# NVlabs/EmerNeRF

Measured on AMD Instinct MI355X. Metric: train rays/sec (8192-ray batch, 128 samples), higher is better.
Workload: dtype f32

## Files before the change

### emernerf_amd/csrc/mlp_fused.hip

```cpp
#include <type_traits>

#include "common.h"
#include "bf16x3.h"

namespace emer {

constexpr int kNThreads = 512;
constexpr int kNeckChunk = 8;

struct WSrc {
    const float *w;
    int64_t sn, sk;
    int32_t n, k;
};

template <int KS> struct Opd { u32x4 h[KS], m[KS], l[KS]; };

template <int KT>
__device__ __forceinline__ void make_opd(const f32x4 (&in)[KT], Opd<(KT + 1) / 2> &o) {
#pragma unroll
    for (int s = 0; s < (KT + 1) / 2; ++s) {
#pragma unroll
        for (int q = 0; q < 4; ++q) {
            const int t = 2 * s + (q >> 1), e = 2 * (q & 1);
// ... 1414 lines not shown
            } else {
                set_kstep(xo, 0, x[0], x[1]);
#pragma unroll
                for (int p = 0; p < 4; ++p) {
                    a1[p] = *reinterpret_cast<const f32x4 *>(rb + 16 * p + 4 * g);
                    a2[p] = *reinterpret_cast<const f32x4 *>(rb + 64 + 16 * p + 4 * g);
                }
                EMER_RGBW_SB();
                ld_frag6(fb, w1gf, 0, 0); mma_frag6<2>(fa, xo, 0, a1[0], a1[1]);
                set_kstep(xo, 1, x[2], x[3]);
                EMER_RGBW_SB();
                ld_frag6(fa, w0f, 0, 1); mma_frag6<2>(fb, xo, 0, a2[0], a2[1]);
                EMER_RGBW_SB();
                ld_frag6(fb, w1gf, 0, 1); mma_frag6<2>(fa, xo, 0, a1[2], a1[3]);
                EMER_RGBW_SB();
                ld_frag6(fa, w0f, 1, 0); mma_frag6<2>(fb, xo, 0, a2[2], a2[3]);
                EMER_RGBW_SB();
                ld_frag6(fb, w1gf, 1, 0); mma_frag6<2>(fa, xo, 1, a1[0], a1[1]);
                EMER_RGBW_SB();
                ld_frag6(fa, w0f, 1, 1); mma_frag6<2>(fb, xo, 1, a2[0], a2[1]);
                {
                    f32x4 v[2] = {a1[0], a1[1]};
                    relu<2>(v);
                    a1[0] = v[0]; a1[1] = v[1];
                    set_kstep(ho, 0, v[0], v[1]);
                }
                EMER_RGBW_SB();
                ld_frag6(fb, w1gf, 1, 1); mma_frag6<2>(fa, xo, 1, a1[2], a1[3]);
                EMER_RGBW_SB();
                ld_frag6(fa, w1af, 0, 0); mma_frag6<2>(fb, xo, 1, a2[2], a2[3]);
                {
                    f32x4 v[2] = {a1[2], a1[3]};
                    relu<2>(v);
                    a1[2] = v[0]; a1[3] = v[1];
                    set_kstep(ho, 1, v[0], v[1]);
                }
                EMER_RGBW_SB();
                ld_frag6(fb, w1af, 0, 1); mma_frag6<2>(fa, ho, 0, a2[0], a2[1]);
                Bq[2] = block32(to_rows<2>(xo, 0, sel), to_rows<2>(xo, 1, sel));
                EMER_RGBW_SB();
                ld_frag6(fa, w1af, 1, 0); mma_frag6<2>(fb, ho, 0, a2[2], a2[3]);
                Bq[3] = block32(to_rows<2>(xo, 2, sel), to_rows<2>(xo, 3, sel));
                EMER_RGBW_SB();
                ld_frag6(fb, w1af, 1, 1); mma_frag6<2>(fa, ho, 1, a2[0], a2[1]);
                Bq[0] = block32(to_rows<2>(ho, 0, sel), to_rows<2>(ho, 1, sel));
                EMER_RGBW_SB();
                ld_frag6(fa, L.w1a, 0, 0); mma_frag6<2>(fb, ho, 1, a2[2], a2[3]);
                Bq[1] = block32(to_rows<2>(ho, 2, sel), to_rows<2>(ho, 3, sel));
                EMER_RGBW_SB();
            }
            relu<4>(a2);
            Opd<2> d1o, d0o;
            f32x4 dg[4];
            rgb_w_chain(st, L, fa, fb, wfirst, d2, a2,
                        [&](f32x4 (&m1)[4]) {
#pragma unroll
                            for (int p = 0; p < 4; ++p) m1[p] = a1[p];
                        },
                        [](int) {}, d1o, d0o, dg);
#pragma unroll
            for (int p = 0; p < 4; ++p) dgp[p] = dg[p];
            dgeo_prev = dgeo;
            EMER_RGBW_SB();
            rgb_w_products(st, sel, d1o, d0o, Bq, s1c, s0c);
        }
        rgb_w_store_sums(a, L, ray, s1c, s0c);
        rpar ^= 1;
    }
    rgb_w_store_dgeo(dgeo_prev, dgp, L.lo64);
    rgb_w_epilogue(st, a, L, smem);
}

struct DensBwdWArgs {
    const float *ddens, *dens, *enc; int64_t n; int32_t n_levels;
    WSrc w0; const float *b0; const float *w1;
    float *denc;
    float *partials; int64_t stride;
};
constexpr int kDensPartMax = 64 * 16 + 64 + 64 + 4;

template <int KS4>
__global__ __launch_bounds__(kNThreads, 2) void density_bwdw_kernel(const DensBwdWArgs a, int32_t F) {
    __shared__ float part[kNThreads / 64][kDensPartMax];
    const int wave = __builtin_amdgcn_readfirstlane(threadIdx.x >> 6), lane = threadIdx.x & 63, m = lane & 15, g = lane >> 4;
    const int32_t K0 = a.w0.k;
    float aw[4][KS4];
    int64_t koff[KS4];
#pragma unroll
    for (int s = 0; s < KS4; ++s) {
        const int32_t k = 4 * s + g, kc = k < K0 ? k : K0 - 1;
        koff[s] = (int64_t)(kc / F) * a.n * F + kc % F;
#pragma unroll
        for (int p = 0; p < 4; ++p) aw[p][s] = k < K0 ? a.w0.w[(int64_t)(16 * p + m) * a.w0.sn + (int64_t)k * a.w0.sk] : 0.0f;
    }
    f32x4 b0r[4], w1r[4], awt[4];
#pragma unroll
    for (int p = 0; p < 4; ++p)
#pragma unroll
        for (int i = 0; i < 4; ++i) {
            const int32_t nf = 16 * p + 4 * g + i;
            b0r[p][i] = a.b0 ? a.b0[nf] : 0.0f;
            w1r[p][i] = a.w1[nf];
            awt[p][i] = m < K0 ? a.w0.w[(int64_t)nf * a.w0.sn + (int64_t)m * a.w0.sk] : 0.0f;
        }
    float w0acc[4 * KS4], w1acc = 0.0f, b0acc = 0.0f, b1acc = 0.0f;
#pragma unroll
    for (int k = 0; k < 4 * KS4; ++k) w0acc[k] = 0.0f;
    const int64_t n_tiles = (a.n + 15) >> 4, n_chunks = (n_tiles + kNeckChunk - 1) / kNeckChunk;
    for (int64_t c = (int64_t)blockIdx.x * (blockDim.x >> 6) + wave; c < n_chunks; c += (int64_t)gridDim.x * (blockDim.x >> 6)) {
        const int64_t t0 = c * kNeckChunk;
        float x[kNeckChunk][KS4], dd[kNeckChunk], de[kNeckChunk];
#pragma unroll
        for (int j = 0; j < kNeckChunk; ++j) {
            const int64_t row = (t0 + j) * 16 + m, rc = row < a.n ? row : a.n - 1;
#pragma unroll
            for (int s = 0; s < KS4; ++s) x[j][s] = a.enc[koff[s] + rc * F];
            dd[j] = a.ddens[rc];
            de[j] = a.dens[rc];
        }
#pragma unroll
        for (int j = 0; j < kNeckChunk; ++j) {
            if (t0 + j >= n_tiles) break;
            const int64_t row = (t0 + j) * 16 + m;
            const bool ok = row < a.n;
            f32x4 h[4];
#pragma unroll
            for (int p = 0; p < 4; ++p) h[p] = b0r[p];
#pragma unroll
            for (int s = 0; s < KS4; ++s)
#pragma unroll
                for (int p = 0; p < 4; ++p) h[p] = __builtin_amdgcn_mfma_f32_16x16x4f32(aw[p][s], x[j][s], h[p], 0, 0, 0);
            relu<4>(h);
            const float fix = ok ? trunc_exp_bwd(dd[j], de[j]) : 0.0f;
            f32x4 dh[4];
#pragma unroll
            for (int p = 0; p < 4; ++p)
#pragma unroll
                for (int i = 0; i < 4; ++i) dh[p][i] = h[p][i] > 0.0f ? w1r[p][i] * fix : 0.0f;
            f32x4 dx = {0.0f, 0.0f, 0.0f, 0.0f};
#pragma unroll
            for (int p = 0; p < 4; ++p)
#pragma unroll
                for (int i = 0; i < 4; ++i) dx = __builtin_amdgcn_mfma_f32_16x16x4f32(awt[p][i], dh[p][i], dx, 0, 0, 0);
            if (ok)
#pragma unroll
                for (int r = 0; r < 4; ++r) {
                    const int32_t k = 4 * g + r;
                    if (k < K0) a.denc[(int64_t)(k / F) * a.n * F + row * F + k % F] = dx[r];
                }
            w1acc += row16_reduce_scatter(h, fix, m);
            b0acc += row16_reduce_scatter(dh, 1.0f, m);
            if (g == 0) b1acc += fix;
#pragma unroll
            for (int k = 0; k < 4 * KS4; ++k) {
                const float ek = __shfl(x[j][k >> 2], 16 * (k & 3) + m, 64);
                w0acc[k] += row16_reduce_scatter(dh, ek, m);
                __builtin_amdgcn_sched_barrier(0);
            }
        }
    }
    const int nf = 16 * (m >> 2) + 4 * g + (m & 3);
#pragma unroll
    for (int k = 0; k < 4 * KS4; ++k)
        if (k < K0) part[wave][nf * K0 + k] = w0acc[k];
    part[wave][64 * K0 + nf] = b0acc;
    part[wave][64 * K0 + 64 + nf] = w1acc;
    b1acc = row16_sum(b1acc);
    if (lane == 0) part[wave][64 * K0 + 128] = b1acc;
    __syncthreads();
    const int total = 64 * K0 + 129;
    for (int i = threadIdx.x; i < total; i += (int)blockDim.x) {
        float t = 0.0f;
        for (int w = 0; w < (int)(blockDim.x >> 6); ++w) t += part[w][i];
        a.partials[(int64_t)blockIdx.x * a.stride + i] = t;
    }
}

struct RMlpFwdArgs {
    const float *x; int64_t ldx;
    int64_t n; int32_t n_levels, k0, n_out, final_act;
    WSrc w0, w1, w2; const float *b0, *b1, *b2;
    float *h1, *h2;
    float *out; int64_t ldo;
};

template <int KT>
__device__ __forceinline__ void ld_rm_k(const float *rowp, bool ok, int g, int k0, f32x4 (&v)[KT]) {
#pragma unroll
    for (int t = 0; t < KT; ++t)
        v[t] = (ok && 16 * t + 4 * g < k0) ? *reinterpret_cast<const f32x4 *>(rowp + t * 16 + 4 * g) : f32x4{0.0f, 0.0f, 0.0f, 0.0f};
}
template <int KT>
__device__ __forceinline__ void st_rm_k(float *rowp, bool ok, int g, int k0, const f32x4 (&v)[KT]) {
    if (!ok) return;
#pragma unroll
    for (int t = 0; t < KT; ++t)
        if (16 * t + 4 * g < k0) *reinterpret_cast<f32x4 *>(rowp + t * 16 + 4 * g) = v[t];
}
template <int NT>
__device__ __forceinline__ void ld_narrow(const float *rowp, bool ok, int g, int n_valid, f32x4 (&v)[NT]) {
#pragma unroll
    for (int p = 0; p < NT; ++p)
#pragma unroll
        for (int i = 0; i < 4; ++i) v[p][i] = (ok && 16 * p + 4 * g + i < n_valid) ? rowp[16 * p + 4 * g + i] : 0.0f;
}
template <int NT>
__device__ __forceinline__ void st_narrow(float *rowp, bool ok, int g, int n_valid, const f32x4 (&v)[NT]) {
    if (!ok) return;
#pragma unroll
    for (int p = 0; p < NT; ++p)
#pragma unroll
        for (int i = 0; i < 4; ++i)
            if (16 * p + 4 * g + i < n_valid) rowp[16 * p + 4 * g + i] = v[p][i];
}

template <int KT0, int NL, int NTO>
struct RMlpFwdLds {
    static constexpr int KS0 = (KT0 + 1) / 2, NP1 = NL == 3 ? 4 : NTO;
    static constexpr int w0 = 0, w1 = w0 + w3_units(4, KS0), w2 = w1 + w3_units(NP1, 2), fl = w2 + (NL == 3 ? w3_units(NTO, 2) : 0);
    static constexpr int b0 = 0, b1 = b0 + 64, b2 = b1 + 64, n_fl = b2 + 64;
    static constexpr size_t bytes = (size_t)fl * 16 + n_fl * sizeof(float);
};

template <int KT0, int F, int NL, int NTO>
__global__ __launch_bounds__(kNThreads, 4) void rmlp_fwd_kernel(const RMlpFwdArgs a) {
    extern __shared__ __attribute__((aligned(16))) u32x4 smem[];
    using Lds = RMlpFwdLds<KT0, NL, NTO>;
    constexpr int KS0 = Lds::KS0, NP1 = Lds::NP1;
    u32x4 *w0l = smem + Lds::w0, *w1l = smem + Lds::w1, *w2l = smem + Lds::w2;
    float *fl = reinterpret_cast<float *>(smem + Lds::fl), *b0l = fl + Lds::b0, *b1l = fl + Lds::b1, *b2l = fl + Lds::b2;
    stage_w3(w0l, 4, KS0, a.w0);
    stage_w3(w1l, NP1, 2, a.w1);
    if (NL == 3) stage_w3(w2l, NTO, 2, a.w2);
    stage_b(b0l, 64, a.b0, a.w0.n);
    stage_b(b1l, 64, a.b1, a.w1.n);
    if (NL == 3) stage_b(b2l, 64, a.b2, a.w2.n);
    __syncthreads();
    const int wave = __builtin_amdgcn_readfirstlane(threadIdx.x >> 6), lane = threadIdx.x & 63, m = lane & 15, g = lane >> 4;
    const W3 w0p = w3_at(w0l, 4, KS0, lane), w1p = w3_at(w1l, NP1, 2, lane), w2p = w3_at(w2l, NTO, 2, lane);
    const bool wide_out = (a.n_out & 3) == 0 && (a.ldo & 3) == 0;
    auto load_x = [&](int64_t row, f32x4 (&v)[KT0]) {
        if constexpr (F == 0) ld_rm_k<KT0>(a.x + row * a.ldx, row < a.n, g, a.k0, v);
        else ld_lm<KT0, F>(a.x, a.n, a.n_levels, row, row < a.n, g, v);
    };
    const int64_t n_tiles = (a.n + 15) >> 4, n_chunks = (n_tiles + kNeckChunk - 1) / kNeckChunk;
    for (int64_t c = (int64_t)blockIdx.x * (blockDim.x >> 6) + wave; c < n_chunks; c += (int64_t)gridDim.x * (blockDim.x >> 6)) {
        const int64_t t0 = c * kNeckChunk;
        f32x4 xn[KT0];
        load_x(t0 * 16 + m, xn);
// ... 489 lines not shown
        };
        return n_out == 1 ? go(I<1>{}) : n_out == 64 ? go(I<4>{}) : go(I<8>{});
    });
}

extern "C" int emer_neck_bwd(const float *d0, const float *d1, const float *ddens, const float *dens, const float *h1,
                             int32_t n_levels, int32_t n_feat, int64_t n, const float *w0, const float *w1, int32_t n_out,
                             float *dpre1, float *dcol0, float *dpre0, float *denc_lm, void *stream) {
    EMER_REQUIRE(n >= 0, "neck_bwd: negative n");
    if (n == 0) return EMER_OK;
    EMER_REQUIRE(emer_neck_supported(n_levels, n_feat, 64, n_out), "neck_bwd: unsupported shape L=%d F=%d n_out=%d", n_levels, n_feat, n_out);
    EMER_REQUIRE(h1 && w0 && w1 && dpre0 && denc_lm, "neck_bwd: null pointer");
    EMER_REQUIRE(!ddens || dens, "neck_bwd: ddens needs the saved density");
    EMER_REQUIRE(n_out != 1 || (ddens && !d0 && !d1), "neck_bwd: density mode takes ddens only");
    const int k0 = n_levels * n_feat;
    NeckBwdArgs a;
    a.d0 = d0; a.d1 = d1; a.ddens = ddens; a.dens = dens; a.h1 = h1; a.n = n; a.n_levels = n_levels;
    a.dpre1 = dpre1; a.dcol0 = dcol0; a.dpre0 = dpre0; a.denc = denc_lm;
    a.w0t = WSrc{w0, 1, k0, k0, 64};
    hipStream_t st = as_stream(stream);
    const uint32_t grid = row_chunk_grid(n);
    const int kt1 = n_out == 1 ? 0 : (n_out == 64 || !d1) ? 4 : 8;
    a.w1t = w_view_t(w1, 64, kt1 == 0 ? 1 : 16 * kt1, 64);
    return dispatch_kt0_f<1, 1, 2, 4, 8>(k0, n_feat, [&](auto kt0, auto f) {
        auto go = [&](auto k1) {
            return launch(neck_bwd_kernel<RUNG(kt0), RUNG(f), RUNG(k1)>, grid, kNThreads, NeckBwdLds<RUNG(kt0), RUNG(k1)>::bytes, st, "neck_bwd", a);
        };
        return kt1 == 0 ? go(I<0>{}) : kt1 == 4 ? go(I<4>{}) : go(I<8>{});
    });
}

static inline uint32_t neck_bwdw_grid(int64_t n, int no) { return persistent_grid((n + 15) / 16, neckw_threads(0, no) / 64, 256); }
static constexpr size_t neck_bwdw_lds(int kt0, int no) {
    const size_t w = (size_t)(w3_units(kt0, 2) + w3_units(4, 2 * no) + w3_units(4, (kt0 + 1) / 2)) * 16
                     + (size_t)(64 + (neckw_threads(kt0, no) / 64) * (1024 * no + 384 * kt0)) * sizeof(float);
    const size_t r = (size_t)(64 * no * 65 + 64 * 16 * kt0 + 64) * sizeof(float);
    return w > r ? w : r;
}
static inline int64_t neck_bwdw_stride(int k0, int n_out) { return (int64_t)n_out * 65 + 64 * (int64_t)k0 + 64; }

extern "C" int emer_neck_bwd_fused_supported(int32_t n_levels, int32_t n_feat, int32_t hidden, int32_t n_out) {
    return (emer_neck_supported(n_levels, n_feat, hidden, n_out) && (n_out == 64 || n_out == 128)) ? 1 : 0;
}
static inline bool neck_bwdw_fits(int32_t n_levels, int32_t n_feat, int64_t n) { return n * n_levels * n_feat < (1ll << 30); }
extern "C" int64_t emer_neck_bwd_fused_workspace(int32_t n_levels, int32_t n_feat, int64_t n, int32_t n_out) {
    if (n <= 0 || !emer_neck_bwd_fused_supported(n_levels, n_feat, 64, n_out) || !neck_bwdw_fits(n_levels, n_feat, n)) return 0;
    return (int64_t)neck_bwdw_grid(n, n_out / 64) * neck_bwdw_stride(n_levels * n_feat, n_out);
}
extern "C" int emer_neck_bwd_fused(const float *d0, const float *d1, const float *ddens, const float *dens, const float *enc_lm,
                                   int32_t n_levels, int32_t n_feat, int64_t n, const float *w0, const float *b0, const float *w1, int32_t n_out,
                                   float *denc_lm, float *workspace, float *dw0, int64_t ld_dw0, float *db0, float *dw1, int64_t ld_dw1,
                                   float *db1, void *stream) {
    EMER_REQUIRE(n >= 0, "neck_bwd_fused: negative n");
    if (n == 0) return EMER_OK;
    EMER_REQUIRE(emer_neck_bwd_fused_supported(n_levels, n_feat, 64, n_out), "neck_bwd_fused: unsupported shape L=%d F=%d n_out=%d", n_levels, n_feat, n_out);
    EMER_REQUIRE(neck_bwdw_fits(n_levels, n_feat, n), "neck_bwd_fused: n * L * F must stay below 2^30 (32-bit lane offsets); split the batch or use emer_neck_bwd");
    EMER_REQUIRE(enc_lm && w0 && b0 && w1 && denc_lm && workspace && dw0 && db0 && dw1 && db1, "neck_bwd_fused: null pointer");
    EMER_REQUIRE(!ddens || dens, "neck_bwd_fused: ddens needs the saved density");
    EMER_REQUIRE(!d1 || n_out == 128, "neck_bwd_fused: d1 is the gradient of outputs 64..127 of a 128-output neck");
    const int k0 = n_levels * n_feat;
    EMER_REQUIRE(ld_dw0 >= k0 && ld_dw1 >= 64, "neck_bwd_fused: leading dimension smaller than the row");
    NeckBwdWArgs a;
    a.d0 = d0; a.d1 = d1; a.ddens = ddens; a.dens = dens; a.enc = enc_lm; a.b0 = b0; a.n = n; a.n_levels = n_levels; a.k0 = k0;
    a.w0 = WSrc{w0, k0, 1, 64, k0};
    a.w0t = WSrc{w0, 1, k0, k0, 64};
    a.w1t = WSrc{w1, 1, 64, 64, n_out};
    a.denc = denc_lm; a.partials = workspace; a.stride = neck_bwdw_stride(k0, n_out);
    hipStream_t st = as_stream(stream);
    const int no = n_out / 64;
    const uint32_t grid = neck_bwdw_grid(n, no);
    const int rc = dispatch_kt0_f<1, 1, 2, 4, 8>(k0, n_feat, [&](auto kt0, auto f) {
        auto go = [&](auto nn) {
            return launch(neck_bwdw_kernel<RUNG(kt0), RUNG(f), RUNG(nn)>, grid, neckw_threads(RUNG(kt0), RUNG(nn)), neck_bwdw_lds(RUNG(kt0), RUNG(nn)), st,
                          "neck_bwd_fused", a);
        };
        return no == 1 ? go(I<1>{}) : go(I<2>{});
    });
    if (rc) return rc;
    const DwReduceJob jb[2] = {{0, n_out, 64, dw1, ld_dw1, db1, 0, {0}, {0}, {0}}, {(int64_t)n_out * 65, 64, k0, dw0, ld_dw0, db0, 0, {0}, {0}, {0}}};
    return launch_dw_reduce_multi(workspace, (int32_t)grid, a.stride, 2, jb, st);
}

static inline int64_t dens_bwdw_stride(int k0) { return ((int64_t)64 * k0 + 129 + 3) / 4 * 4; }
extern "C" int64_t emer_density_bwd_fused_workspace(int32_t n_levels, int32_t n_feat, int64_t n) {
    const int k0 = n_levels * n_feat;
    if (n <= 0 || k0 < 1 || k0 > 16 || !emer_neck_supported(n_levels, n_feat, 64, 1)) return 0;
    return (int64_t)row_chunk_grid(n) * dens_bwdw_stride(k0);
}
extern "C" int emer_density_bwd_fused(const float *ddens, const float *dens, const float *enc_lm, int32_t n_levels, int32_t n_feat, int64_t n,
                                      const float *w0, const float *b0, const float *w1, float *denc_lm, float *workspace, float *dw0,
                                      int64_t ld_dw0, float *db0, float *dw1, float *db1, void *stream) {
    EMER_REQUIRE(n >= 0, "density_bwd_fused: negative n");
    if (n == 0) return EMER_OK;
    const int k0 = n_levels * n_feat;
    EMER_REQUIRE(emer_density_bwd_fused_workspace(n_levels, n_feat, n) > 0, "density_bwd_fused: unsupported shape L=%d F=%d (needs L F <= 16)", n_levels, n_feat);
    EMER_REQUIRE(ddens && dens && enc_lm && w0 && w1 && denc_lm && workspace && dw0 && db0 && dw1 && db1 && ld_dw0 >= k0, "density_bwd_fused: bad arguments");
    DensBwdWArgs a;
    a.ddens = ddens; a.dens = dens; a.enc = enc_lm; a.n = n; a.n_levels = n_levels;
    a.w0 = WSrc{w0, k0, 1, 64, k0};
    a.b0 = b0; a.w1 = w1; a.denc = denc_lm; a.partials = workspace; a.stride = dens_bwdw_stride(k0);
    hipStream_t st = as_stream(stream);
    const uint32_t grid = row_chunk_grid(n);
    if (int rc = pick4<1>((k0 + 3) / 4, [&](auto ks4) { return launch(density_bwdw_kernel<RUNG(ks4)>, grid, kNThreads, 0, st, "density_bwd_fused", a, n_feat); }))
        return rc;
    const DwReduceJob jb[2] = {{0, 64, k0, dw0, ld_dw0, db0, 0, {0}, {0}, {0}}, {64 * k0 + 64, 1, 64, dw1, 64, db1, 0, {0}, {0}, {0}}};
    return launch_dw_reduce_multi(workspace, (int32_t)grid, a.stride, 2, jb, st);
}

extern "C" int emer_rgb_head_fwd(const float *geo, int64_t ld_geo, const float *rb0, const float *rb1, int64_t ld_rb, int64_t n_rays,
                                 int32_t samples_per_ray, int32_t kh, const float *w0, const float *w1, const float *w2,
                                 const float *b2, float *a1, float *a2, float *out, void *stream) {
    EMER_REQUIRE(n_rays >= 0 && samples_per_ray >= 16 && samples_per_ray % 16 == 0 && kh >= 0, "rgb_head_fwd: bad sizes (S must be a multiple of 16)");
    if (n_rays == 0) return EMER_OK;
    EMER_REQUIRE(geo && rb0 && rb1 && w0 && w1 && w2 && (a2 == nullptr || a1 != nullptr) && out && ld_geo >= 64 && ld_geo % 4 == 0 && ld_rb >= 64 && ld_rb % 4 == 0,
                 "rgb_head_fwd: bad arguments");
    RgbFwdArgs a;
    a.geo = geo; a.ld_geo = ld_geo; a.rb0 = rb0; a.rb1 = rb1; a.ld_rb = ld_rb; a.tiles_per_ray = samples_per_ray / 16; a.n_rays = n_rays;
    const RgbViews v = rgb_views(w0, w1, w2, kh, false);
    a.w0g = v.w0g; a.w1a = v.w1a; a.w1g = v.w1g; a.w2 = v.w2;
    a.b2 = b2; a.a1 = a1; a.a2 = a2; a.out = out;
    return launch(rgb_fwd_kernel, ray_grid(n_rays), kNThreads, RgbFwdLds::bytes, as_stream(stream), "rgb_head_fwd", a);
}

extern "C" int emer_field_fwd_supported(int32_t n_levels, int32_t n_feat) {
    const int k0 = n_levels * n_feat;
    return ((n_feat == 2 || n_feat == 4) && k0 >= 1 && k0 <= 64) ? 1 : 0;
}

extern "C" int emer_field_fwd(const float *enc_lm, int32_t n_levels, int32_t n_feat, int64_t n_rays, int32_t samples_per_ray,
                              const float *nw0, const float *nb0, const float *nw1, const float *nb1, const float *rb0, const float *rb1,
                              int64_t ld_rb, int32_t kh, const float *w0, const float *w1, const float *w2, const float *b2, float *geo,
                              float *dens, float *a1, float *a2, float *out, void *stream) {
    EMER_REQUIRE(n_rays >= 0 && samples_per_ray >= 16 && samples_per_ray % 16 == 0 && kh >= 0, "field_fwd: bad sizes (S must be a multiple of 16)");
    if (n_rays == 0) return EMER_OK;
    EMER_REQUIRE(emer_field_fwd_supported(n_levels, n_feat), "field_fwd: unsupported encoding L=%d F=%d", n_levels, n_feat);
    EMER_REQUIRE(enc_lm && nw0 && nw1 && rb0 && rb1 && w0 && w1 && w2 && geo && dens && out && (a2 == nullptr || a1 != nullptr) &&
                 ld_rb >= 64 && ld_rb % 4 == 0, "field_fwd: bad arguments");
    const int64_t n = n_rays * samples_per_ray;
    const int k0 = n_levels * n_feat;
    EMER_REQUIRE(n * k0 < ((int64_t)1 << 30), "field_fwd: n * L * F must stay below 2^30 (32-bit lane offsets)");
    FieldFwdArgs a;
    a.enc = enc_lm; a.n = n; a.n_levels = n_levels;
    a.nw0 = WSrc{nw0, k0, 1, 64, k0};
    a.nw1 = WSrc{nw1, 64, 1, 64, 64};
    a.nb0 = nb0; a.nb1 = nb1; a.geo = geo; a.dens = dens;
    a.r.geo = nullptr; a.r.ld_geo = 64; a.r.rb0 = rb0; a.r.rb1 = rb1; a.r.ld_rb = ld_rb; a.r.tiles_per_ray = samples_per_ray / 16; a.r.n_rays = n_rays;
    const RgbViews v = rgb_views(w0, w1, w2, kh, false);
    a.r.w0g = v.w0g; a.r.w1a = v.w1a; a.r.w1g = v.w1g; a.r.w2 = v.w2;
    a.r.b2 = b2; a.r.a1 = a1; a.r.a2 = a2; a.r.out = out;
    hipStream_t st = as_stream(stream);
    const uint32_t grid = persistent_grid(n_rays, kFieldThreads / 64, 256);
    return dispatch_kt0_f<1, 2, 4>(k0, n_feat, [&](auto kt0, auto f) {
        return launch(field_fwd_kernel<RUNG(kt0), RUNG(f)>, grid, kFieldThreads, FieldFwdLds<RUNG(kt0)>::bytes, st, "field_fwd", a);
    });
}

extern "C" int emer_rgb_head_bwd(const float *dout, const float *out, const float *a1, const float *a2, int64_t n_rays,
                                 int32_t samples_per_ray, int32_t kh, const float *w0, const float *w1, const float *w2,
                                 float *dpre2, float *dpre1, float *dpre0, float *dgeo, float *s1, float *s0, float *workspace,
                                 float *dw2, int64_t ld_dw2, float *db2, void *stream) {
    EMER_REQUIRE(n_rays >= 0 && samples_per_ray >= 16 && samples_per_ray % 16 == 0 && kh >= 0, "rgb_head_bwd: bad sizes (S must be a multiple of 16)");
    if (n_rays == 0) return EMER_OK;
    EMER_REQUIRE(dout && out && a1 && a2 && w0 && w1 && w2 && dpre2 && dpre1 && dpre0 && dgeo && s1 && s0, "rgb_head_bwd: null pointer");
    EMER_REQUIRE(!dw2 || (workspace && ld_dw2 >= 64), "rgb_head_bwd: dw2 needs emer_rgb_head_bwd_workspace floats of workspace and ld_dw2 >= 64");
    RgbBwdArgs a;
    a.dout = dout; a.out = out; a.a1 = a1; a.a2 = a2; a.tiles_per_ray = samples_per_ray / 16; a.n_rays = n_rays;
    const RgbViews v = rgb_views(w0, w1, w2, kh, true);
    a.w2t = v.w2; a.w1at = v.w1a; a.w1gt = v.w1g; a.w0gt = v.w0g;
    a.dpre2 = dpre2; a.dpre1 = dpre1; a.dpre0 = dpre0; a.dgeo = dgeo; a.s1 = s1; a.s0 = s0;
    a.w2part = dw2 ? workspace : nullptr;
    const uint32_t grid = ray_grid(n_rays);
    if (int rc = launch(rgb_bwd_kernel, grid, kNThreads, RgbBwdLds::bytes, as_stream(stream), "rgb_head_bwd", a)) return rc;
    if (dw2) return launch_dw_reduce(workspace, (int32_t)grid, 196, 3, 64, dw2, ld_dw2, db2, as_stream(stream));
    return EMER_OK;
}

static inline uint32_t rgb_bwdw_grid(int64_t n_rays) { return persistent_grid(n_rays, kRWThreads / 64, 256); }
static constexpr int64_t kRgbBwdWStride = 64 * 128 + 64 * 64 + 196;
extern "C" int emer_rgb_head_bwd_fused_supported(int32_t samples_per_ray) {
    return (samples_per_ray >= 16 && samples_per_ray % 16 == 0) ? 1 : 0;
}

extern "C" int64_t emer_rgb_head_bwd_fused_workspace(int64_t n_rays, int32_t samples_per_ray) {
    if (n_rays <= 0 || !emer_rgb_head_bwd_fused_supported(samples_per_ray)) return 0;
    return (int64_t)rgb_bwdw_grid(n_rays) * kRgbBwdWStride;
// ... 202 lines not shown
```

### emernerf_amd/csrc/sampler.hip

```cpp
#include "common.h"

#pragma clang fp contract(off)

#include "contract.h"

namespace emer {

__host__ __device__ __forceinline__ float stot_fwd_map(int type, float t) {
    if (type == EMER_STOT_UNIFORM_LINDISP) return t < 200.0f ? t / 400.0f : 1.0f - 1.0f / (2.0f * t / 200.0f);
    if (type == EMER_STOT_LINDISP) return 1.0f / t;
    if (type == EMER_STOT_SQRT) return sqrtf(t);
    if (type == EMER_STOT_LOG) return logf(t);
    if (type == EMER_STOT_UNIFORM_LINDISP_0) return t < 1.0f ? t / 2.0f : 1.0f - 1.0f / (2.0f * t);
    return t;
}
__device__ __forceinline__ float stot_inv_map(int type, float s) {
    if (type == EMER_STOT_UNIFORM_LINDISP) return s < 0.5f ? s * 400.0f : (1.0f / (2.0f - 2.0f * s)) * 200.0f;
    if (type == EMER_STOT_LINDISP) return 1.0f / s;
    if (type == EMER_STOT_SQRT) return s * s;
    if (type == EMER_STOT_LOG) return expf(s);
    if (type == EMER_STOT_UNIFORM_LINDISP_0) return s < 0.5f ? 2.0f * s : 1.0f / (2.0f - 2.0f * s);
    return s;
}
__device__ __forceinline__ float stot_apply(int type, float s, float s_min, float s_max) {
    return stot_inv_map(type, s * s_max + (1.0f - s) * s_min);
}

constexpr int kRaysPerBlock = 4;

__global__ __launch_bounds__(256) void importance_sample_kernel(const float *__restrict__ vals, const float *__restrict__ cdfs,
                                                                int64_t R, int32_t m, int32_t n,
                                                                const float *__restrict__ jitter, float *__restrict__ s_out,
                                                                float *__restrict__ t_out, float *__restrict__ t_ends, float s_min, float s_max, int type) {
    extern __shared__ __attribute__((aligned(16))) float smem[];
    const int wave = threadIdx.x >> 6, lane = threadIdx.x & 63;
    const int64_t r = (int64_t)blockIdx.x * kRaysPerBlock + wave;
    float *c = smem + (size_t)wave * 2 * m, *v = c + m;
    if (r < R) {
        for (int i = lane; i < m; i += kWave) { c[i] = cdfs[r * m + i]; v[i] = vals[r * m + i]; }
    }
    __syncthreads();
    if (r >= R) return;
    const float c0 = c[0], cl = c[m - 1];
    const float step = (cl - c0) / (float)(n + 1);
    const float beta = jitter ? jitter[r] : 0.5f;
    for (int k = lane; k <= n; k += kWave) {
        const float u = c0 + ((float)k + beta) * step;
        int lo = 0, hi = m;
        while (lo < hi) {
            const int mid = (lo + hi) >> 1;
            if (c[mid] <= u) lo = mid + 1; else hi = mid;
        }
        const int p0 = lo > 0 ? lo - 1 : 0, p1 = lo < m ? lo : m - 1;
        const float cp = c[p0], cq = c[p1], vp = v[p0], vq = v[p1];
        const float d = cq - cp;
        float s;
        if (d < 1e-10f) s = (vp + vq) * 0.5f;
        else s = (u - cp) * ((vq - vp) / d) + vp;
        const int64_t o = r * (int64_t)(n + 1) + k;
        s_out[o] = s;
        if (t_out) {
            const float t = stot_apply(type, s, s_min, s_max);
            if (t_ends) {
                if (k < n) t_out[r * (int64_t)n + k] = t;
                if (k > 0) t_ends[r * (int64_t)n + k - 1] = t;
            } else {
                t_out[o] = t;
            }
        }
    }
}

__global__ __launch_bounds__(256) void importance_sample_points_kernel(const float *__restrict__ vals, const float *__restrict__ cdfs, int64_t R,
                                                                       int32_t m, int32_t n, const float *__restrict__ jitter,
                                                                       float *__restrict__ s_out, float *__restrict__ t_out,
                                                                       float *__restrict__ t_ends, float s_min, float s_max, int type,
                                                                       const float *__restrict__ origins, const float *__restrict__ dirs,
                                                                       const float *__restrict__ aabb, int unbounded,
                                                                       float *__restrict__ normed, float *__restrict__ positions) {
    extern __shared__ __attribute__((aligned(16))) float smem[];
    const int wave = threadIdx.x >> 6, lane = threadIdx.x & 63;
    const int64_t r = (int64_t)blockIdx.x * kRaysPerBlock + wave;
    float *c = smem + (size_t)wave * (2 * m + n + 1), *v = c + m, *te = v + m;
    if (r < R) {
        for (int i = lane; i < m; i += kWave) { c[i] = cdfs[r * m + i]; v[i] = vals[r * m + i]; }
    }
    __syncthreads();
    if (r >= R) return;
    const float c0 = c[0], cl = c[m - 1];
    const float step = (cl - c0) / (float)(n + 1);
    const float beta = jitter ? jitter[r] : 0.5f;
    for (int k = lane; k <= n; k += kWave) {
        const float u = c0 + ((float)k + beta) * step;
        int lo = 0, hi = m;
        while (lo < hi) {
            const int mid = (lo + hi) >> 1;
            if (c[mid] <= u) lo = mid + 1; else hi = mid;
        }
        const int p0 = lo > 0 ? lo - 1 : 0, p1 = lo < m ? lo : m - 1;
        const float cp = c[p0], cq = c[p1], vp = v[p0], vq = v[p1];
        const float d = cq - cp;
        float s;
        if (d < 1e-10f) s = (vp + vq) * 0.5f;
        else s = (u - cp) * ((vq - vp) / d) + vp;
        s_out[r * (int64_t)(n + 1) + k] = s;
        const float t = stot_apply(type, s, s_min, s_max);
        te[k] = t;
        if (k < n) t_out[r * (int64_t)n + k] = t;
        if (k > 0) t_ends[r * (int64_t)n + k - 1] = t;
    }
    __builtin_amdgcn_fence(__ATOMIC_ACQ_REL, "wavefront");
    const Aabb bb = load_aabb(aabb);
    for (int k = lane; k < n; k += kWave) {
        const float tsum = te[k] + te[k + 1];
        float p[3], q[3];
        ray_point(origins + r * 3, dirs + r * 3, tsum, p);
        contract_point(bb, unbounded != 0, p, q);
        const int64_t i = r * (int64_t)n + k;
        normed[i * 3] = q[0]; normed[i * 3 + 1] = q[1]; normed[i * 3 + 2] = q[2];
        if (positions) { positions[i * 3] = p[0]; positions[i * 3 + 1] = p[1]; positions[i * 3 + 2] = p[2]; }
    }
}

__global__ __launch_bounds__(256) void stot_kernel(const float *__restrict__ s, int64_t n, float s_min, float s_max, int type,
                                                   float *__restrict__ t) {
    for (int64_t i = (int64_t)blockIdx.x * 256 + threadIdx.x; i < n; i += (int64_t)gridDim.x * 256)
        t[i] = stot_apply(type, s[i], s_min, s_max);
}

}

using namespace emer;

extern "C" int emer_importance_sample(const float *vals, const float *cdfs, int64_t R, int32_t m, int32_t n,
                                      const float *jitter, float *s_out, float *t_out, float *t_ends, float t_min,
                                      float t_max, int stot_type, void *stream) {
    EMER_REQUIRE(R >= 0 && n >= 1, "importance_sample: bad sizes R=%lld n=%d", (long long)R, n);
    EMER_REQUIRE(m >= 2 && m <= 4096, "importance_sample: m=%d edges per ray not in 2..4096", m);
    if (R == 0) return EMER_OK;
    EMER_REQUIRE(vals && cdfs && s_out, "importance_sample: null pointer");
    EMER_REQUIRE(!t_ends || t_out, "importance_sample: t_ends needs t_out (the interval starts)");
    EMER_REQUIRE(stot_type >= 0 && stot_type <= 5, "importance_sample: unknown stot_type %d", stot_type);
    const float s_min = stot_fwd_map(stot_type, t_min), s_max = stot_fwd_map(stot_type, t_max);
    const size_t lds = (size_t)kRaysPerBlock * 2 * m * sizeof(float);
    if (int rc = reserve_lds(reinterpret_cast<const void *>(importance_sample_kernel), lds, "importance_sample")) return rc;
    hipLaunchKernelGGL(importance_sample_kernel, dim3((uint32_t)ceil_div(R, kRaysPerBlock)), dim3(256), lds, as_stream(stream),
                       vals, cdfs, R, m, n, jitter, s_out, t_out, t_ends, s_min, s_max, stot_type);
    return check_launch("importance_sample");
}

extern "C" int64_t emer_importance_sample_points_capacity(void) {
    int dev = 0, bytes = 0;
    if (hipGetDevice(&dev) != hipSuccess || hipDeviceGetAttribute(&bytes, hipDeviceAttributeMaxSharedMemoryPerBlock, dev) != hipSuccess) return 0;
    return (int64_t)bytes / (kRaysPerBlock * (int64_t)sizeof(float));
}

extern "C" int emer_importance_sample_points(const float *vals, const float *cdfs, int64_t R, int32_t m, int32_t n, const float *jitter,
                                             float *s_out, float *t_starts, float *t_ends, float t_min, float t_max, int stot_type,
                                             const float *origins, const float *dirs, const float *aabb, int unbounded, float *normed,
                                             float *positions, void *stream) {
    EMER_REQUIRE(R >= 0 && n >= 1, "importance_sample_points: bad sizes R=%lld n=%d", (long long)R, n);
    EMER_REQUIRE(m >= 2 && m <= 4096 && 2 * (int64_t)m + n + 1 <= emer_importance_sample_points_capacity(),
                 "importance_sample_points: m=%d edges, n=%d intervals per ray do not fit the LDS", m, n);
    if (R == 0) return EMER_OK;
    EMER_REQUIRE(vals && cdfs && s_out && t_starts && t_ends && origins && dirs && aabb && normed, "importance_sample_points: null pointer");
    EMER_REQUIRE(stot_type >= 0 && stot_type <= 5, "importance_sample_points: unknown stot_type %d", stot_type);
    const float s_min = stot_fwd_map(stot_type, t_min), s_max = stot_fwd_map(stot_type, t_max);
    const size_t lds = (size_t)kRaysPerBlock * (2 * (size_t)m + n + 1) * sizeof(float);
    if (int rc = reserve_lds(reinterpret_cast<const void *>(importance_sample_points_kernel), lds, "importance_sample_points")) return rc;
    hipLaunchKernelGGL(importance_sample_points_kernel, dim3((uint32_t)ceil_div(R, kRaysPerBlock)), dim3(256), lds, as_stream(stream), vals, cdfs,
                       R, m, n, jitter, s_out, t_starts, t_ends, s_min, s_max, stot_type, origins, dirs, aabb, unbounded, normed, positions);
    return check_launch("importance_sample_points");
}

extern "C" int emer_stot(const float *s, int64_t n, float t_min, float t_max, int stot_type, float *t, void *stream) {
    EMER_REQUIRE(n >= 0, "stot: negative n");
    if (n == 0) return EMER_OK;
    EMER_REQUIRE(s && t, "stot: null pointer");
    EMER_REQUIRE(stot_type >= 0 && stot_type <= 5, "stot: unknown stot_type %d", stot_type);
    const float s_min = stot_fwd_map(stot_type, t_min), s_max = stot_fwd_map(stot_type, t_max);
    const uint32_t blocks = (uint32_t)(ceil_div(n, 256) < 2048 ? ceil_div(n, 256) : 2048);
    hipLaunchKernelGGL(stot_kernel, dim3(blocks), dim3(256), 0, as_stream(stream), s, n, s_min, s_max, stot_type, t);
    return check_launch("stot");
}
```

Measured before the change: 3.600 million.

## Compute density weight gradients with MFMA outer products and cache LDS capacity query

The density backward kernel's weight-gradient accumulation stops using per-element cross-lane reduce-scatter shuffles. It recomputes the hidden layer transposed and accumulates dW0 through MFMA outer products, with b0 and w1 broadcast from LDS instead of held in registers. The grid moves to a persistent-grid helper, and the sampler caches the device LDS size per device so each call skips a HIP attribute query. The cost is extra MFMA work for the transposed recompute, added LDS traffic and a block-wide barrier.

```diff
diff --git a/emernerf_amd/csrc/mlp_fused.hip b/emernerf_amd/csrc/mlp_fused.hip
--- a/emernerf_amd/csrc/mlp_fused.hip
+++ b/emernerf_amd/csrc/mlp_fused.hip
@@ -1520,6 +1520,7 @@
 template <int KS4>
 __global__ __launch_bounds__(kNThreads, 2) void density_bwdw_kernel(const DensBwdWArgs a, int32_t F) {
     __shared__ float part[kNThreads / 64][kDensPartMax];
+    __shared__ f32x4 bw[32], b0q[64];
     const int wave = __builtin_amdgcn_readfirstlane(threadIdx.x >> 6), lane = threadIdx.x & 63, m = lane & 15, g = lane >> 4;
     const int32_t K0 = a.w0.k;
     float aw[4][KS4];
@@ -1531,19 +1532,21 @@
 #pragma unroll
         for (int p = 0; p < 4; ++p) aw[p][s] = k < K0 ? a.w0.w[(int64_t)(16 * p + m) * a.w0.sn + (int64_t)k * a.w0.sk] : 0.0f;
     }
-    f32x4 b0r[4], w1r[4], awt[4];
+    f32x4 awt[4];
 #pragma unroll
     for (int p = 0; p < 4; ++p)
 #pragma unroll
-        for (int i = 0; i < 4; ++i) {
-            const int32_t nf = 16 * p + 4 * g + i;
-            b0r[p][i] = a.b0 ? a.b0[nf] : 0.0f;
-            w1r[p][i] = a.w1[nf];
-            awt[p][i] = m < K0 ? a.w0.w[(int64_t)nf * a.w0.sn + (int64_t)m * a.w0.sk] : 0.0f;
-        }
-    float w0acc[4 * KS4], w1acc = 0.0f, b0acc = 0.0f, b1acc = 0.0f;
-#pragma unroll
-    for (int k = 0; k < 4 * KS4; ++k) w0acc[k] = 0.0f;
+        for (int i = 0; i < 4; ++i) awt[p][i] = m < K0 ? a.w0.w[(int64_t)(16 * p + 4 * g + i) * a.w0.sn + (int64_t)m * a.w0.sk] : 0.0f;
+    if (threadIdx.x < 64) {
+        const float b = a.b0 ? a.b0[threadIdx.x] : 0.0f;
+        reinterpret_cast<float *>(bw)[threadIdx.x] = b;
+        reinterpret_cast<float *>(bw)[64 + threadIdx.x] = a.w1[threadIdx.x];
+        b0q[threadIdx.x] = f32x4{b, b, b, b};
+    }
+    __syncthreads();
+    f32x4 w0acc[4];
+    float w1acc[4] = {0.0f, 0.0f, 0.0f, 0.0f}, b0acc[4] = {0.0f, 0.0f, 0.0f, 0.0f}, b1acc = 0.0f;
+    zero<4>(w0acc);
     const int64_t n_tiles = (a.n + 15) >> 4, n_chunks = (n_tiles + kNeckChunk - 1) / kNeckChunk;
     for (int64_t c = (int64_t)blockIdx.x * (blockDim.x >> 6) + wave; c < n_chunks; c += (int64_t)gridDim.x * (blockDim.x >> 6)) {
         const int64_t t0 = c * kNeckChunk;
@@ -1561,9 +1564,11 @@
             if (t0 + j >= n_tiles) break;
             const int64_t row = (t0 + j) * 16 + m;
             const bool ok = row < a.n;
+            int og = g, om = m;
+            asm volatile("" : "+v"(og), "+v"(om));
             f32x4 h[4];
 #pragma unroll
-            for (int p = 0; p < 4; ++p) h[p] = b0r[p];
+            for (int p = 0; p < 4; ++p) h[p] = bw[4 * p + og];
 #pragma unroll
             for (int s = 0; s < KS4; ++s)
 #pragma unroll
@@ -1572,9 +1577,11 @@
             const float fix = ok ? trunc_exp_bwd(dd[j], de[j]) : 0.0f;
             f32x4 dh[4];
 #pragma unroll
-            for (int p = 0; p < 4; ++p)
-#pragma unroll
-                for (int i = 0; i < 4; ++i) dh[p][i] = h[p][i] > 0.0f ? w1r[p][i] * fix : 0.0f;
+            for (int p = 0; p < 4; ++p) {
+                const f32x4 w1r = bw[16 + 4 * p + og];
+#pragma unroll
+                for (int i = 0; i < 4; ++i) dh[p][i] = h[p][i] > 0.0f ? w1r[i] * fix : 0.0f;
+            }
             f32x4 dx = {0.0f, 0.0f, 0.0f, 0.0f};
 #pragma unroll
             for (int p = 0; p < 4; ++p)
@@ -1586,23 +1593,41 @@
                     const int32_t k = 4 * g + r;
                     if (k < K0) a.denc[(int64_t)(k / F) * a.n * F + row * F + k % F] = dx[r];
                 }
-            w1acc += row16_reduce_scatter(h, fix, m);
-            b0acc += row16_reduce_scatter(dh, 1.0f, m);
             if (g == 0) b1acc += fix;
-#pragma unroll
-            for (int k = 0; k < 4 * KS4; ++k) {
-                const float ek = __shfl(x[j][k >> 2], 16 * (k & 3) + m, 64);
-                w0acc[k] += row16_reduce_scatter(dh, ek, m);
-                __builtin_amdgcn_sched_barrier(0);
-            }
-        }
-    }
-    const int nf = 16 * (m >> 2) + 4 * g + (m & 3);
-#pragma unroll
-    for (int k = 0; k < 4 * KS4; ++k)
-        if (k < K0) part[wave][nf * K0 + k] = w0acc[k];
-    part[wave][64 * K0 + nf] = b0acc;
-    part[wave][64 * K0 + 64 + nf] = w1acc;
+            __builtin_amdgcn_sched_barrier(0);
+            f32x4 xr = {0.0f, 0.0f, 0.0f, 0.0f};
+#pragma unroll
+            for (int s = 0; s < KS4; ++s) xr = __builtin_amdgcn_mfma_f32_16x16x4f32(x[j][s], m == 4 * s + g ? 1.0f : 0.0f, xr, 0, 0, 0);
+            float fr[4];
+#pragma unroll
+            for (int r = 0; r < 4; ++r) fr[r] = __shfl(fix, 4 * g + r, 64);
+#pragma unroll
+            for (int p = 0; p < 4; ++p) {
+                const float w1t = reinterpret_cast<const float *>(bw)[64 + 16 * p + om];
+                f32x4 ht = b0q[16 * p + om];
+#pragma unroll
+                for (int s = 0; s < KS4; ++s) ht = __builtin_amdgcn_mfma_f32_16x16x4f32(x[j][s], aw[p][s], ht, 0, 0, 0);
+#pragma unroll
+                for (int r = 0; r < 4; ++r) {
+                    const bool on = ht[r] > 0.0f;
+                    const float dht = on ? w1t * fr[r] : 0.0f;
+                    w1acc[p] += (on ? ht[r] : 0.0f) * fr[r];
+                    b0acc[p] += dht;
+                    w0acc[p] = __builtin_amdgcn_mfma_f32_16x16x4f32(dht, xr[r], w0acc[p], 0, 0, 0);
+                }
+            }
+        }
+    }
+#pragma unroll
+    for (int p = 0; p < 4; ++p) {
+#pragma unroll
+        for (int r = 0; r < 4; ++r)
+            if (m < K0) part[wave][(16 * p + 4 * g + r) * K0 + m] = w0acc[p][r];
+        float b = b0acc[p], w = w1acc[p];
+        b += __shfl_xor(b, 16, 64); b += __shfl_xor(b, 32, 64);
+        w += __shfl_xor(w, 16, 64); w += __shfl_xor(w, 32, 64);
+        if (g == 0) { part[wave][64 * K0 + 16 * p + m] = b; part[wave][64 * K0 + 64 + 16 * p + m] = w; }
+    }
     b1acc = row16_sum(b1acc);
     if (lane == 0) part[wave][64 * K0 + 128] = b1acc;
     __syncthreads();
@@ -2258,10 +2283,11 @@
 }
 
 static inline int64_t dens_bwdw_stride(int k0) { return ((int64_t)64 * k0 + 129 + 3) / 4 * 4; }
+static inline uint32_t dens_bwdw_grid(int64_t n) { return persistent_grid(((n + 15) / 16 + kNeckChunk - 1) / kNeckChunk, kNThreads / 64, 256); }
 extern "C" int64_t emer_density_bwd_fused_workspace(int32_t n_levels, int32_t n_feat, int64_t n) {
     const int k0 = n_levels * n_feat;
     if (n <= 0 || k0 < 1 || k0 > 16 || !emer_neck_supported(n_levels, n_feat, 64, 1)) return 0;
-    return (int64_t)row_chunk_grid(n) * dens_bwdw_stride(k0);
+    return (int64_t)dens_bwdw_grid(n) * dens_bwdw_stride(k0);
 }
 extern "C" int emer_density_bwd_fused(const float *ddens, const float *dens, const float *enc_lm, int32_t n_levels, int32_t n_feat, int64_t n,
                                       const float *w0, const float *b0, const float *w1, float *denc_lm, float *workspace, float *dw0,
@@ -2276,7 +2302,7 @@
     a.w0 = WSrc{w0, k0, 1, 64, k0};
     a.b0 = b0; a.w1 = w1; a.denc = denc_lm; a.partials = workspace; a.stride = dens_bwdw_stride(k0);
     hipStream_t st = as_stream(stream);
-    const uint32_t grid = row_chunk_grid(n);
+    const uint32_t grid = dens_bwdw_grid(n);
     if (int rc = pick4<1>((k0 + 3) / 4, [&](auto ks4) { return launch(density_bwdw_kernel<RUNG(ks4)>, grid, kNThreads, 0, st, "density_bwd_fused", a, n_feat); }))
         return rc;
     const DwReduceJob jb[2] = {{0, 64, k0, dw0, ld_dw0, db0, 0, {0}, {0}, {0}}, {64 * k0 + 64, 1, 64, dw1, 64, db1, 0, {0}, {0}, {0}}};
diff --git a/emernerf_amd/csrc/sampler.hip b/emernerf_amd/csrc/sampler.hip
--- a/emernerf_amd/csrc/sampler.hip
+++ b/emernerf_amd/csrc/sampler.hip
@@ -1,4 +1,7 @@
 #include "common.h"
+
+#include <map>
+#include <mutex>
 
 #pragma clang fp contract(off)
 
@@ -149,10 +152,24 @@
     return check_launch("importance_sample");
 }
 
+static int points_capacity(int64_t *floats) {
+    static std::mutex mu;
+    static std::map<int, int64_t> known;
+    int dev = 0, bytes = 0;
+    hipError_t e = hipGetDevice(&dev);
+    if (e == hipSuccess) {
+        std::lock_guard<std::mutex> lock(mu);
+        const auto it = known.find(dev);
+        if (it != known.end()) { *floats = it->second; return EMER_OK; }
+        e = hipDeviceGetAttribute(&bytes, hipDeviceAttributeMaxSharedMemoryPerBlock, dev);
+        if (e == hipSuccess) { *floats = known[dev] = (int64_t)bytes / (kRaysPerBlock * (int64_t)sizeof(float)); return EMER_OK; }
+    }
+    emer::set_error("importance_sample_points: cannot ask device %d for its LDS size: %s", dev, hipGetErrorString(e));
+    return EMER_E_LAUNCH;
+}
 extern "C" int64_t emer_importance_sample_points_capacity(void) {
-    int dev = 0, bytes = 0;
-    if (hipGetDevice(&dev) != hipSuccess || hipDeviceGetAttribute(&bytes, hipDeviceAttributeMaxSharedMemoryPerBlock, dev) != hipSuccess) return 0;
-    return (int64_t)bytes / (kRaysPerBlock * (int64_t)sizeof(float));
+    int64_t floats = 0;
+    return points_capacity(&floats) == EMER_OK ? floats : 0;
 }
 
 extern "C" int emer_importance_sample_points(const float *vals, const float *cdfs, int64_t R, int32_t m, int32_t n, const float *jitter,
@@ -160,8 +177,9 @@
                                              const float *origins, const float *dirs, const float *aabb, int unbounded, float *normed,
                                              float *positions, void *stream) {
     EMER_REQUIRE(R >= 0 && n >= 1, "importance_sample_points: bad sizes R=%lld n=%d", (long long)R, n);
-    EMER_REQUIRE(m >= 2 && m <= 4096 && 2 * (int64_t)m + n + 1 <= emer_importance_sample_points_capacity(),
-                 "importance_sample_points: m=%d edges, n=%d intervals per ray do not fit the LDS", m, n);
+    int64_t cap = 0;
+    if (int rc = points_capacity(&cap)) return rc;
+    EMER_REQUIRE(m >= 2 && m <= 4096 && 2 * (int64_t)m + n + 1 <= cap, "importance_sample_points: m=%d edges, n=%d intervals per ray do not fit the LDS", m, n);
     if (R == 0) return EMER_OK;
     EMER_REQUIRE(vals && cdfs && s_out && t_starts && t_ends && origins && dirs && aabb && normed, "importance_sample_points: null pointer");
     EMER_REQUIRE(stot_type >= 0 && stot_type <= 5, "importance_sample_points: unknown stot_type %d", stot_type);
```

After: 3.616 million (median of 3 runs). About the same (+0.4%).

## Compute density backward weight gradients with transposed MFMA and prefetch tiles

Applied to the files above, without the earlier changes.

The density backward-weight kernel now recomputes the hidden activations in transposed layout with MFMA. It accumulates dW0 via MFMA outer products instead of per-k shuffles and row16 reduce-scatter, which removes many cross-lane reductions per tile. Bias and w1 are staged in LDS and read through an opaque SGPR offset to limit register pressure. Encoding tiles are software-prefetched a few tiles ahead across chunk boundaries, and the grid changes to a persistent size. The costs are doubled forward MFMA work, extra transposed loads, and more live registers.

```diff
diff --git a/emernerf_amd/csrc/mlp_fused.hip b/emernerf_amd/csrc/mlp_fused.hip
--- a/emernerf_amd/csrc/mlp_fused.hip
+++ b/emernerf_amd/csrc/mlp_fused.hip
@@ -1531,39 +1531,59 @@
 #pragma unroll
         for (int p = 0; p < 4; ++p) aw[p][s] = k < K0 ? a.w0.w[(int64_t)(16 * p + m) * a.w0.sn + (int64_t)k * a.w0.sk] : 0.0f;
     }
-    f32x4 b0r[4], w1r[4], awt[4];
+    __shared__ __attribute__((aligned(16))) float bw[128];
+    if (threadIdx.x < 128) bw[threadIdx.x] = threadIdx.x < 64 ? (a.b0 ? a.b0[threadIdx.x] : 0.0f) : a.w1[threadIdx.x - 64];
+    __syncthreads();
+    const f32x4 *bwl = reinterpret_cast<const f32x4 *>(bw) + g;
+    f32x4 awt[4];
 #pragma unroll
     for (int p = 0; p < 4; ++p)
 #pragma unroll
         for (int i = 0; i < 4; ++i) {
             const int32_t nf = 16 * p + 4 * g + i;
-            b0r[p][i] = a.b0 ? a.b0[nf] : 0.0f;
-            w1r[p][i] = a.w1[nf];
             awt[p][i] = m < K0 ? a.w0.w[(int64_t)nf * a.w0.sn + (int64_t)m * a.w0.sk] : 0.0f;
         }
-    float w0acc[4 * KS4], w1acc = 0.0f, b0acc = 0.0f, b1acc = 0.0f;
-#pragma unroll
-    for (int k = 0; k < 4 * KS4; ++k) w0acc[k] = 0.0f;
+    const int32_t mc = m < K0 ? m : K0 - 1;
+    const int64_t kofft = (int64_t)(mc / F) * a.n * F + mc % F;
+    f32x4 w0acc[4];
+    zero<4>(w0acc);
+    float w1acc[4] = {0.0f, 0.0f, 0.0f, 0.0f}, b0acc[4] = {0.0f, 0.0f, 0.0f, 0.0f}, b1acc = 0.0f;
+    constexpr int kAhead = KS4 <= 2 ? 4 : 2;
     const int64_t n_tiles = (a.n + 15) >> 4, n_chunks = (n_tiles + kNeckChunk - 1) / kNeckChunk;
-    for (int64_t c = (int64_t)blockIdx.x * (blockDim.x >> 6) + wave; c < n_chunks; c += (int64_t)gridDim.x * (blockDim.x >> 6)) {
+    const int64_t c_step = (int64_t)gridDim.x * (blockDim.x >> 6);
+    float x[kNeckChunk][KS4], xt[kNeckChunk][4], dd[kNeckChunk], de[kNeckChunk];
+    auto ld_tile = [&](int slot, int64_t tile) {
+        const int64_t row = tile * 16 + m, rc = row < a.n ? row : a.n - 1;
+#pragma unroll
+        for (int s = 0; s < KS4; ++s) x[slot][s] = a.enc[koff[s] + rc * F];
+        dd[slot] = a.ddens[rc];
+        de[slot] = a.dens[rc];
+#pragma unroll
+        for (int r = 0; r < 4; ++r) {
+            const int64_t rowt = tile * 16 + 4 * g + r, rct = rowt < a.n ? rowt : a.n - 1;
+            xt[slot][r] = a.enc[kofft + rct * F];
+        }
+    };
+    int64_t c = (int64_t)blockIdx.x * (blockDim.x >> 6) + wave;
+    if (c < n_chunks) {
+#pragma unroll
+        for (int j = 0; j < kAhead; ++j) ld_tile(j, c * kNeckChunk + j);
+    }
+    for (; c < n_chunks; c += c_step) {
         const int64_t t0 = c * kNeckChunk;
-        float x[kNeckChunk][KS4], dd[kNeckChunk], de[kNeckChunk];
-#pragma unroll
-        for (int j = 0; j < kNeckChunk; ++j) {
-            const int64_t row = (t0 + j) * 16 + m, rc = row < a.n ? row : a.n - 1;
-#pragma unroll
-            for (int s = 0; s < KS4; ++s) x[j][s] = a.enc[koff[s] + rc * F];
-            dd[j] = a.ddens[rc];
-            de[j] = a.dens[rc];
-        }
 #pragma unroll
         for (int j = 0; j < kNeckChunk; ++j) {
             if (t0 + j >= n_tiles) break;
+            ld_tile((j + kAhead) % kNeckChunk, j + kAhead < kNeckChunk ? t0 + j + kAhead : (c + c_step) * kNeckChunk + (j + kAhead - kNeckChunk));
             const int64_t row = (t0 + j) * 16 + m;
             const bool ok = row < a.n;
+            int z;
+            asm volatile("s_mov_b32 %0, 0" : "=s"(z));
+            const f32x4 *b0l = bwl + z, *w1l = b0l + 16;
+            const float *bsl = bw + m + z;
             f32x4 h[4];
 #pragma unroll
-            for (int p = 0; p < 4; ++p) h[p] = b0r[p];
+            for (int p = 0; p < 4; ++p) h[p] = b0l[4 * p];
 #pragma unroll
             for (int s = 0; s < KS4; ++s)
 #pragma unroll
@@ -1572,9 +1592,11 @@
             const float fix = ok ? trunc_exp_bwd(dd[j], de[j]) : 0.0f;
             f32x4 dh[4];
 #pragma unroll
-            for (int p = 0; p < 4; ++p)
-#pragma unroll
-                for (int i = 0; i < 4; ++i) dh[p][i] = h[p][i] > 0.0f ? w1r[p][i] * fix : 0.0f;
+            for (int p = 0; p < 4; ++p) {
+                const f32x4 w1v = w1l[4 * p];
+#pragma unroll
+                for (int i = 0; i < 4; ++i) dh[p][i] = h[p][i] > 0.0f ? w1v[i] * fix : 0.0f;
+            }
             f32x4 dx = {0.0f, 0.0f, 0.0f, 0.0f};
 #pragma unroll
             for (int p = 0; p < 4; ++p)
@@ -1586,23 +1608,41 @@
                     const int32_t k = 4 * g + r;
                     if (k < K0) a.denc[(int64_t)(k / F) * a.n * F + row * F + k % F] = dx[r];
                 }
-            w1acc += row16_reduce_scatter(h, fix, m);
-            b0acc += row16_reduce_scatter(dh, 1.0f, m);
             if (g == 0) b1acc += fix;
-#pragma unroll
-            for (int k = 0; k < 4 * KS4; ++k) {
-                const float ek = __shfl(x[j][k >> 2], 16 * (k & 3) + m, 64);
-                w0acc[k] += row16_reduce_scatter(dh, ek, m);
-                __builtin_amdgcn_sched_barrier(0);
-            }
-        }
-    }
-    const int nf = 16 * (m >> 2) + 4 * g + (m & 3);
-#pragma unroll
-    for (int k = 0; k < 4 * KS4; ++k)
-        if (k < K0) part[wave][nf * K0 + k] = w0acc[k];
-    part[wave][64 * K0 + nf] = b0acc;
-    part[wave][64 * K0 + 64 + nf] = w1acc;
+            float fx[4];
+#pragma unroll
+            for (int r = 0; r < 4; ++r) fx[r] = __shfl(fix, 4 * g + r, 64);
+#pragma unroll
+            for (int p = 0; p < 4; ++p) {
+                const float b0t = bsl[16 * p], w1t = bsl[64 + 16 * p];
+                f32x4 ht = {b0t, b0t, b0t, b0t}, dht;
+#pragma unroll
+                for (int s = 0; s < KS4; ++s) ht = __builtin_amdgcn_mfma_f32_16x16x4f32(x[j][s], aw[p][s], ht, 0, 0, 0);
+#pragma unroll
+                for (int r = 0; r < 4; ++r) {
+                    const bool on = ht[r] > 0.0f;
+                    dht[r] = on ? w1t * fx[r] : 0.0f;
+                    w1acc[p] += on ? ht[r] * fx[r] : 0.0f;
+                    b0acc[p] += dht[r];
+                }
+#pragma unroll
+                for (int r = 0; r < 4; ++r) w0acc[p] = __builtin_amdgcn_mfma_f32_16x16x4f32(dht[r], xt[j][r], w0acc[p], 0, 0, 0);
+            }
+        }
+    }
+#pragma unroll
+    for (int p = 0; p < 4; ++p) {
+#pragma unroll
+        for (int r = 0; r < 4; ++r)
+            if (m < K0) part[wave][(16 * p + 4 * g + r) * K0 + m] = w0acc[p][r];
+        float b = b0acc[p], w = w1acc[p];
+        b += __shfl_xor(b, 16, 64); b += __shfl_xor(b, 32, 64);
+        w += __shfl_xor(w, 16, 64); w += __shfl_xor(w, 32, 64);
+        if (g == 0) {
+            part[wave][64 * K0 + 16 * p + m] = b;
+            part[wave][64 * K0 + 64 + 16 * p + m] = w;
+        }
+    }
     b1acc = row16_sum(b1acc);
     if (lane == 0) part[wave][64 * K0 + 128] = b1acc;
     __syncthreads();
@@ -2258,10 +2298,11 @@
 }
 
 static inline int64_t dens_bwdw_stride(int k0) { return ((int64_t)64 * k0 + 129 + 3) / 4 * 4; }
+static inline uint32_t dens_bwdw_grid(int64_t n) { return persistent_grid(((n + 15) / 16 + kNeckChunk - 1) / kNeckChunk, kNThreads / 64, 256); }
 extern "C" int64_t emer_density_bwd_fused_workspace(int32_t n_levels, int32_t n_feat, int64_t n) {
     const int k0 = n_levels * n_feat;
     if (n <= 0 || k0 < 1 || k0 > 16 || !emer_neck_supported(n_levels, n_feat, 64, 1)) return 0;
-    return (int64_t)row_chunk_grid(n) * dens_bwdw_stride(k0);
+    return (int64_t)dens_bwdw_grid(n) * dens_bwdw_stride(k0);
 }
 extern "C" int emer_density_bwd_fused(const float *ddens, const float *dens, const float *enc_lm, int32_t n_levels, int32_t n_feat, int64_t n,
                                       const float *w0, const float *b0, const float *w1, float *denc_lm, float *workspace, float *dw0,
@@ -2276,7 +2317,7 @@
     a.w0 = WSrc{w0, k0, 1, 64, k0};
     a.b0 = b0; a.w1 = w1; a.denc = denc_lm; a.partials = workspace; a.stride = dens_bwdw_stride(k0);
     hipStream_t st = as_stream(stream);
-    const uint32_t grid = row_chunk_grid(n);
+    const uint32_t grid = dens_bwdw_grid(n);
     if (int rc = pick4<1>((k0 + 3) / 4, [&](auto ks4) { return launch(density_bwdw_kernel<RUNG(ks4)>, grid, kNThreads, 0, st, "density_bwd_fused", a, n_feat); }))
         return rc;
     const DwReduceJob jb[2] = {{0, 64, k0, dw0, ld_dw0, db0, 0, {0}, {0}, {0}}, {64 * k0 + 64, 1, 64, dw1, 64, db1, 0, {0}, {0}, {0}}};
```

Result: no change. 3.569 million before, 3.589 million after (median of 6 runs) (+0.6%).
